# wangty537/raft_optical_flow

Hardware: AMD Instinct MI355X
Metric: image-pairs/s at Sintel 436x1024, 32 iters; corr-lookup GB/s vs HBM peak (higher is better)
Workload: dtype fp32 (convs: f16x3 split MFMA, fp32 accumulate); 1 GPU; RAFT-full inference, 436x1024 padded to 440x1024, 1 pair(s)/GPU/step, iters=32, all-pairs corr, hipGraph; global_batch=1, parallelism=frame-pair sharding x1

## Files before the change

include/raft_hip.h:

```cpp
#ifndef RAFT_HIP_H_
#define RAFT_HIP_H_

#include <stddef.h>

#ifdef __cplusplus
extern "C" {
#endif

#define RAFT_HIP_ABI_VERSION 19

#define RAFT_E_INVALID (-1)
#define RAFT_E_ALIGN (-2)

typedef void* raft_stream_t;

int raft_hip_abi_version(void);
const char* raft_hip_arch(void);
const char* raft_hip_last_error(void);
const char* raft_hip_source_hash(void);
int raft_debug_launch_span(int enable);
int raft_debug_launch_span_read(unsigned long long* host, int n);
int raft_debug_fill_lds_nan(raft_stream_t stream);

size_t raft_corr_pyramid_floats(int B, int H, int W, int num_levels);
// ... 128 lines not shown
int raft_conv2d_in_norm_ok(const raft_conv2d_params* p);
int raft_instnorm_merge(const float* part, int slots_per_image, int B, int C, int stats_ld, float eps,
                        float* stats, raft_stream_t stream);
size_t raft_instnorm_merge_ws_floats(int slots_per_image, int B, int C);
int raft_instnorm_merge_ws(const float* part, int slots_per_image, int B, int C, int stats_ld, float eps, void* ws,
                           float* stats, raft_stream_t stream);
size_t raft_instnorm_merge_counters(int B, int C);
int raft_instnorm_merge_fused(const float* part, int slots_per_image, int B, int C, int stats_ld, float eps, void* ws,
                              int* counters, float* stats, raft_stream_t stream);

int raft_conv2d_packed_shape(int mode, int n, int kh, int kw, int cin, int* n_pad, int* k_pad);
int raft_conv2d(const raft_conv2d_params* p, raft_stream_t stream);
int raft_conv2d_pair(const raft_conv2d_params* p0, const raft_conv2d_params* p1, raft_stream_t stream);
int raft_conv2d_set_halo_loaders(int nl);
int raft_conv2d_set_halo_ks(int ks);
int raft_conv2d_split_weight(const float* w, void* out, int n_pad, int k_pad, raft_stream_t stream);
size_t raft_conv2d_split_scaled_bytes(int n_pad, int k_pad);
int raft_conv2d_split_weight_scaled(const float* w, void* out, int n_pad, int k_pad, raft_stream_t stream);
int raft_conv2d_split_weight_prec(const float* w, void* out, int n_pad, int k_pad, int precision,
                                  raft_stream_t stream);

size_t raft_instnorm_workspace_floats(int B, int HW, int C);
int raft_instnorm_stats(const float* x, int ld, int B, int HW, int C, float eps, float* stats,
                        float* workspace, raft_stream_t stream);
int raft_groupnorm_stats(const float* x, int ld, int B, int HW, int C, int G, float eps, float* stats,
                         raft_stream_t stream);
int raft_norm_apply_affine(const float* x, int ld, const float* stats, const float* gamma, const float* beta,
                           const float* resid, int resid_ld, const float* resid_stats, const float* resid_gamma,
                           const float* resid_beta, int relu_mode, float* out, int out_ld, int B, int HW, int C,
                           raft_stream_t stream);
// ... 59 lines not shown
```

raft_optical_flow_amd/_lib.py:

```python
from __future__ import annotations

import ctypes
import os
import threading

_HERE = os.path.dirname(os.path.abspath(__file__))
LIB_PATH = os.environ.get("RAFT_HIP_LIB") or os.path.join(_HERE, "libraft_hip.so")

c_int = ctypes.c_int
c_float = ctypes.c_float
c_size_t = ctypes.c_size_t
c_long = ctypes.c_long
c_void_p = ctypes.c_void_p
c_char_p = ctypes.c_char_p
P = c_void_p

RAFT_CONV_VEC = 0
RAFT_CONV_GATHER = 1

PREC_FP32 = 0
PREC_F16X3 = 1
PREC_F16 = 2
PREC_BF16 = 3
PRECISIONS = {"fp32": PREC_FP32, "f16x3": PREC_F16X3, "f16": PREC_F16, "bf16": PREC_BF16}
# ... 125 lines not shown
    "raft_conv2d_stats_slots": (c_int, [ctypes.POINTER(ConvParams)]),
    "raft_conv2d_halo_tile_rows": (c_int, [ctypes.POINTER(ConvParams)]),
    "raft_conv2d_halo_tiles_per_wg": (c_int, [ctypes.POINTER(ConvParams)]),
    "raft_conv2d_form": (c_int, [ctypes.POINTER(ConvParams), ctypes.POINTER(ConvForm)]),
    "raft_conv2d_pair_form": (c_int, [ctypes.POINTER(ConvParams), ctypes.POINTER(ConvParams),
                                      ctypes.POINTER(ConvForm), ctypes.POINTER(c_int)]),
    "raft_debug_launch_span": (c_int, [c_int]),
    "raft_debug_launch_span_read": (c_int, [P, c_int]),
    "raft_conv2d_in_norm_ok": (c_int, [ctypes.POINTER(ConvParams)]),
    "raft_instnorm_merge": (c_int, [P, c_int, c_int, c_int, c_int, c_float, P, P]),
    "raft_instnorm_merge_ws_floats": (c_size_t, [c_int, c_int, c_int]),
    "raft_instnorm_merge_ws": (c_int, [P, c_int, c_int, c_int, c_int, c_float, P, P, P]),
    "raft_instnorm_merge_counters": (c_size_t, [c_int, c_int]),
    "raft_conv2d_set_halo_loaders": (c_int, [c_int]),
    "raft_conv2d_set_halo_ks": (c_int, [c_int]),
    "raft_instnorm_merge_fused": (c_int, [P, c_int, c_int, c_int, c_int, c_float, P, P, P, P]),
    "raft_conv2d_split_weight": (c_int, [P, P, c_int, c_int, P]),
    "raft_conv2d_split_weight_prec": (c_int, [P, P, c_int, c_int, c_int, P]),
    "raft_conv2d_split_scaled_bytes": (c_size_t, [c_int, c_int]),
    "raft_conv2d_split_weight_scaled": (c_int, [P, P, c_int, c_int, P]),
    "raft_instnorm_workspace_floats": (c_size_t, [c_int, c_int, c_int]),
    "raft_instnorm_stats": (c_int, [P, c_int, c_int, c_int, c_int, c_float, P, P, P]),
    "raft_groupnorm_stats": (c_int, [P, c_int, c_int, c_int, c_int, c_int, c_float, P, P]),
    "raft_norm_apply_affine": (c_int, [P, c_int, P, P, P, P, c_int, P, P, P, c_int, P, c_int, c_int, c_int, c_int, P]),
    "raft_instnorm_apply": (c_int, [P, c_int, P, P, c_int, P, c_int, P, c_int, c_int, c_int, c_int, P]),
    "raft_prep_images": (c_int, [P, P, P, c_int, c_int, c_int, P]),
    "raft_init_coords": (c_int, [P, P, c_int, c_int, c_int, P]),
    "raft_flow_from_coords": (c_int, [P, P, c_int, c_int, c_int, P]),
    "raft_convex_upsample": (c_int, [P, P, c_int, P, c_int, c_int, c_int, P]),
    "raft_upflow8": (c_int, [P, P, c_int, c_int, c_int, P]),
# ... 87 lines not shown
```

raft_optical_flow_amd/csrc/conv_common.hpp:

```cpp
#pragma once

#include "common.hpp"

namespace raft {
namespace {

using h4 = __attribute__((ext_vector_type(4))) _Float16;
using v4u = __attribute__((ext_vector_type(4))) unsigned;
using h8 = __attribute__((ext_vector_type(8))) _Float16;
using bf4 = __attribute__((ext_vector_type(4))) __bf16;
using bf8 = __attribute__((ext_vector_type(8))) __bf16;

__device__ __forceinline__ h4 to_bf16x4(const f32x4 x) {
  return __builtin_bit_cast(h4, __builtin_convertvector(x, bf4));
}

constexpr float SPLIT_SCALE = 2048.f;

__device__ __forceinline__ void split4(const f32x4 x, h4& hi, h4& lo) {
#pragma unroll
  for (int e = 0; e < 4; ++e) {
    const _Float16 h = (_Float16)x[e];
    hi[e] = h;
    lo[e] = (_Float16)((x[e] - (float)h) * SPLIT_SCALE);
// ... 134 lines not shown
  for (int j = 0; j < 4; ++j) {
    float x[4] = {v[4 * j], v[4 * j + 1], v[4 * j + 2], v[4 * j + 3]};
    quad_transpose(x);
    const int row = q == 0 ? rows[4 * j] : q == 1 ? rows[4 * j + 1] : q == 2 ? rows[4 * j + 2] : rows[4 * j + 3];
    const unsigned off = row >= 0 ? ((unsigned)row * (unsigned)ld + c0) * 4u : OFF_INVALID;
    __builtin_amdgcn_raw_buffer_store_b128(__builtin_bit_cast(v4u, f32x4{x[0], x[1], x[2], x[3]}), rs,
                                           full ? off : OFF_INVALID, 0, CPOL);
    if (part) {
#pragma unroll
      for (int i = 0; i < 4; ++i)
        if (nq + i < ncols) __builtin_amdgcn_raw_buffer_store_b32(__builtin_bit_cast(unsigned, x[i]), rs, off + 4u * i, 0, CPOL);
    }
  }
}

template <bool WT = false, int R0 = 0, int RN = 16>
__device__ __forceinline__ void tile_epilogue(const raft_conv2d_params& p, const int (&rows)[16], int n,
                                              const f32x16& acc) {
  static_assert(!WT || (R0 == 0 && RN == 16), "write-through epilogues store whole 16-row tiles");
  const bool ncol = n < p.n;
  const int nc = ncol ? n : p.n - 1;
  float v[16];
  const float bias = p.bias ? p.bias[nc] : 0.f;
#pragma unroll
  for (int r = R0; r < R0 + RN; ++r) v[r] = acc[r] + bias;
  if (p.add0) {
    float t[16];
    load_rows<WT, R0, RN>(p.add0, p.add0_ld, rows, nc, t);
#pragma unroll
    for (int r = R0; r < R0 + RN; ++r) v[r] += t[r];
  }
  float* dst = p.out;
  int ld = p.out_ld, col = n;
  const int epi = p.epilogue;
  if (epi == RAFT_EPI_LINEAR) {
#pragma unroll
    for (int r = R0; r < R0 + RN; ++r) v[r] *= p.alpha;
  } else if (epi == RAFT_EPI_RELU) {
#pragma unroll
    for (int r = R0; r < R0 + RN; ++r) v[r] = fmaxf(v[r], 0.f);
  } else if (epi == RAFT_EPI_RESID_RELU) {
    float t[16];
    load_rows<WT, R0, RN>(p.aux0, p.aux0_ld, rows, nc, t);
#pragma unroll
    for (int r = R0; r < R0 + RN; ++r) v[r] = fmaxf(t[r] + fmaxf(v[r], 0.f), 0.f);
  } else if (epi == RAFT_EPI_GRU_ZR) {
    if (nc < p.split) {
#pragma unroll
      for (int r = R0; r < R0 + RN; ++r) v[r] = sigmoid_bf(v[r]);
    } else {
      col = nc - p.split;
      float t[16];
      load_rows<WT, R0, RN>(p.aux0, p.aux0_ld, rows, col, t);
#pragma unroll
      for (int r = R0; r < R0 + RN; ++r) v[r] = sigmoid_bf(v[r]) * t[r];
      dst = p.out1;
      ld = p.out1_ld;
    }
  } else if (epi == RAFT_EPI_GRU_Q) {
    float h[16], z[16];
    load_rows<WT, R0, RN>(p.aux0, p.aux0_ld, rows, nc, h);
    load_rows<WT, R0, RN>(p.aux1, p.aux1_ld, rows, nc, z);
#pragma unroll
    for (int r = R0; r < R0 + RN; ++r) v[r] = (1.0f - z[r]) * h[r] + z[r] * tanh_bf(v[r]);
  } else if (epi == RAFT_EPI_TANH_RELU) {
    if (nc < p.split) {
#pragma unroll
      for (int r = R0; r < R0 + RN; ++r) v[r] = tanh_bf(v[r]);
    } else {
#pragma unroll
      for (int r = R0; r < R0 + RN; ++r) v[r] = fmaxf(v[r], 0.f);
      dst = p.out1;
      ld = p.out1_ld;
      col = n - p.split;
    }
  } else if (epi == RAFT_EPI_ADD_TO_OUT) {
    float t[16];
// ... 7 lines not shown
    for (int r = R0; r < R0 + RN; ++r) big |= ncol && rows[r] >= 0 && fabsf(v[r]) > RAFT_RANGE_LIMIT;
    if (big) *p.range_flag = 1;
  }
  if (WT && (((uintptr_t)dst) & 15) == 0 && (ld & 3) == 0) {
    store_tile16<WT ? CPOL_SC1 : 0>(dst, ld, (long)p.batch * p.out_h * p.out_w, rows, col, n - (threadIdx.x & 3), p.n, v);
    return;
  }
#pragma unroll
  for (int r = R0; r < R0 + RN; ++r)
    if (ncol && rows[r] >= 0) {
      if constexpr (WT)
        __hip_atomic_store(dst + eidx(rows[r], ld, col), v[r], __ATOMIC_RELAXED, __HIP_MEMORY_SCOPE_AGENT);
      else
        dst[eidx(rows[r], ld, col)] = v[r];
    }
}

__device__ __forceinline__ f32x4 tile_stats_vals(const int (&rows)[16], const f32x16& acc, float bias) {
  float s = 0.f, c = 0.f;
#pragma unroll
  for (int r = 0; r < 16; ++r) {
    s += rows[r] >= 0 ? acc[r] + bias : 0.f;
    c += rows[r] >= 0 ? 1.f : 0.f;
  }
  s += __shfl_xor(s, 32);
  c += __shfl_xor(c, 32);
  const float mean = c > 0.f ? s / c : 0.f;
  float m2 = 0.f;
#pragma unroll
  for (int r = 0; r < 16; ++r) {
// ... 66 lines not shown

struct HaloOperands {
  raft_conv2d_params p;
  int k_pad, n_pad;
  unsigned w_bytes, in0_bytes, in1_bytes;
};

using ConvForm = struct raft_conv2d_form;

int conv_halo_launch(const HaloOperands& o, hipStream_t s, ConvForm* form = nullptr);
int conv_halo_launch_pair(const HaloOperands& o0, const HaloOperands& o1, hipStream_t s, ConvForm* form = nullptr);
int conv_stem_launch(const raft_conv2d_params& p, int k_pad, hipStream_t s, ConvForm* form = nullptr);
int conv_halo_stats_slots(const HaloOperands& o);
bool conv_halo_covers(const HaloOperands& o);
int conv_halo_tile_rows(const HaloOperands& o);
int conv_halo_tiles_per_wg(const HaloOperands& o);
bool conv_halo_norm_ok(const HaloOperands& o);
int conv_stem_stats_slots(const raft_conv2d_params& p, int k_pad);

}
```

raft_optical_flow_amd/csrc/conv_gemm.hip:

```cpp
#include "conv_common.hpp"

namespace raft {
namespace {

constexpr int BM = 64;
constexpr int BN = 64;
constexpr int BK = 32;
constexpr int LDSK = BK + 4;
constexpr int STAGE = (BM + BN) * LDSK;
constexpr int MAX_GATHER_K = 1024;
#ifndef CONV_SCHED
#define CONV_SCHED 1
#endif
#ifndef GEMM_NS
#define GEMM_NS 2
#endif

struct ConvArgs {
  raft_conv2d_params p;
  int M;
  int K;
  int ctot;
  int cpad;
  int taps;
// ... 898 lines not shown
extern "C" int raft_conv2d_in_norm_ok(const raft_conv2d_params* pp) {
  ConvArgs a;
  HaloOperands o;
  if (!pp || conv_prepare(pp, a, o)) return 0;
  return pp->mode == RAFT_CONV_VEC && pp->n > 4 && conv_halo_norm_ok(o) ? 1 : 0;
}

extern "C" int raft_conv2d_halo_tile_rows(const raft_conv2d_params* pp) {
  ConvArgs a;
  HaloOperands o;
  if (!pp || conv_prepare(pp, a, o)) return 0;
  if (pp->mode != RAFT_CONV_VEC || small_n(*pp)) return 0;
  return conv_halo_tile_rows(o);
}

extern "C" int raft_conv2d_halo_tiles_per_wg(const raft_conv2d_params* pp) {
  ConvArgs a;
  HaloOperands o;
  if (!pp || conv_prepare(pp, a, o)) return 0;
  if (pp->mode != RAFT_CONV_VEC || small_n(*pp)) return 0;
  return conv_halo_tiles_per_wg(o);
}

extern "C" int raft_conv2d_stats_slots(const raft_conv2d_params* pp) {
  ConvArgs a;
  HaloOperands o;
  if (!pp || conv_prepare(pp, a, o)) return 0;
  const raft_conv2d_params& p = *pp;
  if (p.epilogue != RAFT_EPI_LINEAR || p.alpha != 1.0f || p.add0 || (p.n <= 4 && p.mode == RAFT_CONV_VEC)) return 0;
  if (p.mode == RAFT_CONV_VEC) {
// ... 52 lines not shown
```

raft_optical_flow_amd/csrc/conv_halo.hip:

```cpp
#include <atomic>
#include <type_traits>

#include "conv_common.hpp"

namespace raft {
namespace {

constexpr int HTW = 16;
constexpr int HTH = 8;
constexpr int HTH_BIG = 16;
constexpr int HALO_LDS = 160 * 1024;

struct HaloArgs {
  raft_conv2d_params p;
  const float* inv_scale;
  int K;
  int nch;
  int nk;
  int gn;
  int tx_n, ty_n;
  unsigned w_bytes, in0_bytes, in1_bytes;
};

struct HaloLaunch {
  HaloArgs a[2];
  int sp0, sp1;
  int m;
  int grid0;
};

constexpr int patch_slots(int T, int U, int D, int late = 0) {
  for (int pa = 1; pa < 16; ++pa) {
    bool ok = true;
    for (int c = pa; c < 512 && ok; ++c) {
      const int last = (c - pa) * T + T - 1;
      const int rd = last == 0 ? -1 : (last - 1) / U;
// ... 20 lines not shown
                                                                              : 2;
#else
  static constexpr int D = halo_lds_bytes(T, U, 3, BNT, PI, WR) <= LB ? 3 : 2;
#endif
  static constexpr int PA = patch_slots(T, U, D);
#ifndef HALO_WX
#define HALO_WX 0
#endif
  static constexpr int DW = (T > 1 && D == 3 && HALO_WX > 0 &&
                             U * (D + HALO_WX + 1) * BNT * WR + PA * PI * 1024 + 16 * 1024 <= LB)
                                ? D + HALO_WX
                                : D;
  static constexpr int SB = U * (DW + 1);
  static constexpr int LDS_B = SB * BNT * WR, LDS_A = PA * PI * 1024;
};

#ifdef STAMPS
__device__ unsigned long long g_hstamp[8 * 16384];
__device__ unsigned long long g_lstamp[8 * 16384];
__device__ __forceinline__ unsigned long long hstamp_real() {
  unsigned long long t;
  __builtin_amdgcn_sched_barrier(0);
  asm volatile("s_memrealtime %0\n\ts_waitcnt lgkmcnt(0)" : "=s"(t)::"memory");
  __builtin_amdgcn_sched_barrier(0);
  return t;
}
__device__ __forceinline__ unsigned long long hstamp_now() {
  unsigned long long t;
  __builtin_amdgcn_sched_barrier(0);
  asm volatile("s_memtime %0\n\ts_waitcnt lgkmcnt(0)" : "=s"(t)::"memory");
// ... 50 lines not shown
  constexpr int SGB = (ENC && NL == 8) ? 0 : HALO_SGB;
#ifndef HALO_RELAX
#define HALO_RELAX 1
#endif
  constexpr int NRD1 = NSUB * 2 * (X3 ? 2 : 1) + MF * 2 * (X3 ? 2 : 1);
  constexpr bool RELAX = HALO_RELAX && SGB > 0 && LSPLIT && !MT && patch_slots(T, U, D, 1) == PA && NRD1 <= 15;
  static_assert(D >= 2 && C::LDS_B + C::LDS_A <= C::LB, "LDS budget");
  static_assert(KS == 1 || (KS == 2 && !MT && !ENC && LSPLIT && SGB > 0 && MF == 1 && NSUB <= 2 && (NL == 4 || NL == 8) &&
                            SB % 2 == 0 && 8 * 4096 <= C::LDS_B + C::LDS_A && (DW == D || !KSW) && NBI % NWPC == 0 &&
                            NWPC >= 1),
                "the K-split form: one tile of 32 x 64 blocks on the pre-split path, 4 loaders");
  static_assert(NWP >= 1 && NBI % NWP == 0, "a wave's weight pieces lie in one K-step");
  static_assert(U % 2 == 0 && (T == 1 || T >= U), "fragment parity; at most one chunk start per load set");
  constexpr int NORM_BYTES = halo_norm_bytes<KH, KW, BNT, PREC, ENC>(C::LDS_B, C::LDS_A, D);
  static_assert(NORM_BYTES == 0 || NORM_BYTES >= 256 * 8, "room for one image's norm table");

#ifdef STAMPS
  const unsigned long long r_entry = hstamp_real(), c_entry = hstamp_now();
#endif
  const int lane = threadIdx.x & 63;
  const int w = __builtin_amdgcn_readfirstlane(threadIdx.x >> 6);
  constexpr int NCW = 4 * KS;
  const bool loader = w >= NCW;
  const int lw = loader ? w - NCW : w;
  const int wc = w & 3;
  const int kp = KS > 1 ? (w >> 2) & (KS - 1) : 0;

  const HaloArgs& a = args[prob];
  const raft_conv2d_params& p = a.p;
  const int per = a.tx_n * a.ty_n;
// ... 272 lines not shown
              nnew += pcw;
            }
            if constexpr (DW == D) {
              issue_weights(s + D);
              nnew += NWP;
            }
          }
          wait_vm_n(s + 1 < NS ? nnew : 0);
          __builtin_amdgcn_s_barrier();
        }
        wait_vm<0>();
        if constexpr (KS > 1) __builtin_amdgcn_s_barrier();
        return;
      }
#endif
      constexpr int PMAX = (U * D + T - 1) / T + 1;
      Staged pv[PMAX];
      int pks[PMAX], pcs[PMAX];
      int nst = 0;
#pragma unroll
      for (int u = 0; u < D; ++u) {
        int kt, c;
        if (set_chunk(u, kt, c)) {
#pragma unroll
          for (int k = 0; k < PMAX; ++k)
            if (k == nst) {
              load_patch(kt, c, pv[k]);
              pks[k] = kt;
              pcs[k] = c;
            }
// ... 2 lines not shown
      }
      wait_vm<0>();
#pragma unroll
      for (int k = 0; k < PMAX; ++k)
        if (k < nst) store_patch(pks[k], pcs[k], pv[k]);
      __builtin_amdgcn_s_waitcnt(0xC07F);
      __builtin_amdgcn_s_barrier();
      int pend_k = -1, pend_c = 0;
#ifdef STAMPS
      unsigned long long l_st = 0, l_ld = 0, l_w = 0, l_wait = 0, l_bar = 0, l0 = hstamp_now(), l1;
      const unsigned long long l_loop = l0;
#define LSTAMP(acc) (l1 = hstamp_now(), acc += l1 - l0, l0 = l1)
#else
#define LSTAMP(acc)
#endif
      for (int s = 0; s < NS; ++s) {
        if (pend_k >= 0) {
          wait_vm<LNWP>();
          store_patch(pend_k, pend_c, pv[0]);
          pend_k = -1;
        }
        LSTAMP(l_st);
        int nnew = 0;
        if (s + D < NS) {
          int kt, c;
          if (set_chunk(s + D, kt, c)) {
            load_patch(kt, c, pv[0]);
            pend_k = kt;
            pend_c = c;
            nnew = 2 * TI;
          }
// ... 6 lines not shown
          }
        }
        if constexpr (DW > D && !KSW) {
          if (s + DW < NS) {
            issue_weights(s + DW);
            nnew += NWP;
          }
        }
        LSTAMP(l_w);
        wait_vm_n(s + 1 < NS ? nnew + (DW - D) * NWP : 0);
        __builtin_amdgcn_s_waitcnt(0xC07F);
        LSTAMP(l_wait);
        __builtin_amdgcn_s_barrier();
        LSTAMP(l_bar);
      }
#undef LSTAMP
#ifdef STAMPS
      {
        const unsigned lid = blockIdx.x * NL + lw;
        if (lane == 0 && lid < 16384) {
          unsigned long long* g = g_lstamp + lid * 8;
          g[0] = l_st;
          g[1] = l_ld;
          g[2] = l_w;
          g[3] = l_wait;
          g[4] = l_bar;
          g[5] = hstamp_now() - l_loop;
          g[6] = 1;
        }
      }
// ... 44 lines not shown
    for (int f = 0; f < MF; ++f)
#pragma unroll
      for (int sb = 0; sb < NSUB; ++sb) acc[f][sb] = f32x16{};
#pragma unroll
    for (int f = 0; f < AXF; ++f)
#pragma unroll
      for (int sb = 0; sb < AXS; ++sb) accx[f][sb] = f32x16{};
  };
  clear_acc();
  int b_bs = kp;
  int a_t = 0, a_ky = 0, a_kx = 0, a_ps = 0;
  struct Frag {
    h8 ah[MF][2], al[MF][2];
    h8 bh[NSUB][2], bl[NSUB][2];
  };
  f32x4 av[MF][4];
  auto read_b = [&](Frag& F) {
    const char* Bb = smem + b_bs * (BNT * WROW);
#pragma unroll
    for (int sb = 0; sb < NSUB; ++sb) {
#pragma unroll
      for (int qq = 0; qq < 2; ++qq) {
        F.bh[sb][qq] = *reinterpret_cast<const h8*>(Bb + (cb + sb * 32 + m) * WROW + (((2 * h + qq) ^ bsw) << 4));
        if constexpr (X3)
          F.bl[sb][qq] = *reinterpret_cast<const h8*>(Bb + (cb + sb * 32 + m) * WROW + (((4 + 2 * h + qq) ^ bsw) << 4));
      }
    }
    b_bs = b_bs + KS >= SB ? b_bs + KS - SB : b_bs + KS;
  };
  auto advance_a = [&]() {
// ... 121 lines not shown
#pragma unroll
          for (int r = 0; r < 16; ++r) acc[f][sb][r] += accx[f][sb][r] * (1.0f / SPLIT_SCALE);
    }
    f32x4 stv[NSUB];
    const int oh = __builtin_amdgcn_readfirstlane(p.out_h), ow = __builtin_amdgcn_readfirstlane(p.out_w);
    const int rowb = t.b * oh;
#pragma unroll
    for (int f = 0; f < MF; ++f) {
      int rows[16];
#pragma unroll
      for (int r = 0; r < 16; ++r) {
        const int mm = (r & 3) + 8 * (r >> 2) + 4 * h;
        const int y = t.y0 + 2 * (wm * MF + f) + (mm >> 4), x = t.x0 + (mm & 15);
        rows[r] = ((y < oh) & (x < ow)) ? (rowb + y) * ow + x : -1;
      }
#pragma unroll
      for (int sb = 0; sb < NSUB; ++sb) tile_epilogue<false>(p, rows, t.n0 + cb + sb * 32 + m, acc[f][sb]);
      if constexpr (ENC) {
        if (p.stats_part) {
#pragma unroll
          for (int sb = 0; sb < NSUB; ++sb) {
            const int n = t.n0 + sb * 32 + m;
            const f32x4 v = tile_stats_vals(rows, acc[f][sb], p.bias ? p.bias[n < p.n ? n : 0] : 0.f);
            stv[sb] = f == 0 ? v : stats_combine(stv[sb], v);
            if (f == MF - 1) stats_write(p, n, (long)t.st * 4 + w, stv[sb]);
          }
        }
      }
    }
  };

  auto epilogue_ks2 = [&](const Tile& t) {
// ... 39 lines not shown
      else
        tile_epilogue<false, 0, 8>(p, rows, t.n0 + cb + m, keep);
    } else if constexpr (KS > 1) {
      if constexpr (X3 && !SC) {
#pragma unroll
        for (int sb = 0; sb < NSUB; ++sb)
#pragma unroll
          for (int r = 0; r < 16; ++r) acc[0][sb][r] += accx[0][sb][r] * (1.0f / SPLIT_SCALE);
      }
      f32x16 keep, send;
#pragma unroll
      for (int r = 0; r < 16; ++r) {
        keep[r] = kp ? acc[0][1][r] : acc[0][0][r];
        send[r] = kp ? acc[0][0][r] : acc[0][1][r];
      }
      f32x4* mine = reinterpret_cast<f32x4*>(smem + (wc * 2 + kp) * 4096) + lane * 4;
      const f32x4* theirs = reinterpret_cast<const f32x4*>(smem + (wc * 2 + (kp ^ 1)) * 4096) + lane * 4;
#pragma unroll
      for (int q = 0; q < 4; ++q)
        mine[q ^ (lane & 3)] = f32x4{send[4 * q], send[4 * q + 1], send[4 * q + 2], send[4 * q + 3]};
      __builtin_amdgcn_s_waitcnt(0xC07F);
      __builtin_amdgcn_s_barrier();
#pragma unroll
      for (int q = 0; q < 4; ++q) {
        const f32x4 o = theirs[q ^ (lane & 3)];
#pragma unroll
        for (int i = 0; i < 4; ++i) keep[4 * q + i] += o[i];
      }
      const int oh = __builtin_amdgcn_readfirstlane(p.out_h), ow = __builtin_amdgcn_readfirstlane(p.out_w);
      const int rowb = t.b * oh;
      int rows[16];
#pragma unroll
      for (int r = 0; r < 16; ++r) {
        const int mm = (r & 3) + 8 * (r >> 2) + 4 * h;
        const int y = t.y0 + 2 * wm + (mm >> 4), x = t.x0 + (mm & 15);
        rows[r] = ((y < oh) & (x < ow)) ? (rowb + y) * ow + x : -1;
      }
      tile_epilogue<false>(p, rows, t.n0 + cb + kp * 32 + m, keep);
    }
  };

  if constexpr (KS > 1) {
    if (kp) advance_a();
  }
  const WPiecesC wpc = wpieces_c(KSW ? w : 0);
  if constexpr (KSW) {
#pragma unroll
    for (int u = 0; u < DW; ++u) issue_weights_c(u, wpc);
    wait_vm<NWPC * (DW - 2)>();
  } else if constexpr (KS > 1) {
    if (NL == 8 || kp == 0) {
#pragma unroll
      for (int u = 0; u < DW; ++u) issue_weights(u);
// ... 189 lines not shown
      g[1] = r_exit;
      g[2] = c_loop - c_entry;
      g[3] = t_cmp;
      g[4] = t_wait + t_bar;
      g[5] = t_epi;
      g[6] = c_exit - c_entry;
    }
  }
#endif
}

template <int KH, int KW, int BNT, int PREC, bool ENC = false, int TH = HTH, bool MT = false, int NL = 4, int KS = 1>
__global__ __launch_bounds__(64 * (4 * KS + NL)) void conv_halo_kernel(HaloLaunch hl) {
  using C = HaloCfg<KH, KW, BNT, PREC == RAFT_PREC_F16X3 ? 128 : 64, TH>;
  constexpr int NORM_BYTES = halo_norm_bytes<KH, KW, BNT, PREC, ENC>(C::LDS_B, C::LDS_A, C::D);
  __shared__ __attribute__((aligned(1024))) char smem[C::LDS_B + C::LDS_A + NORM_BYTES];
  int g = xcd_tile(blockIdx.x, gridDim.x);
  const int prob = g >= hl.grid0 ? 1 : 0;
  g -= prob * hl.grid0;
  const int gn = hl.a[prob].gn;
  if constexpr (MT) {
    const int st0 = (g / gn) * hl.m;
    const int ntl = min(hl.m, (prob ? hl.sp1 : hl.sp0) - st0);
    halo_body<KH, KW, BNT, PREC, ENC, TH, true, NL>(hl.a, prob, g % gn, st0, ntl, smem);
  } else {
    halo_body<KH, KW, BNT, PREC, ENC, TH, false, NL, KS>(hl.a, prob, g % gn, g / gn, 1, smem);
  }
}

std::atomic<int> g_halo_nl{0};
bool halo_nl8() {
// ... 9 lines not shown
#define HALO_KS2_NL8 0
#endif
#ifndef HALO_KS2_BN32
#define HALO_KS2_BN32 0
#endif
std::atomic<int> g_halo_ks{0};
bool halo_ks2() {
  int v = g_halo_ks.load(std::memory_order_relaxed);
  if (v == 0) {
    const char* e = getenv("RAFT_HALO_KS2");
    v = e && e[0] == '0' ? 1 : 2;
    g_halo_ks.store(v, std::memory_order_relaxed);
  }
  return v == 2;
}
bool halo_nl8_enc() {
  const char* e = getenv("RAFT_HALO_NL8_ENC");
  return !(e && e[0] == '0');
}
constexpr bool halo_no_mt(int prec, int taps, int bn) { return prec != RAFT_PREC_F16X3 && taps == 9 && bn == 128; }

template <int KH, int KW, int BNT, int PREC, bool ENC, int TH, bool MT, int NL = 4, int KS = 1>
void halo_start(const HaloLaunch& l, dim3 grid, hipStream_t s, ConvForm* q) {
  if (q) {
    *q = ConvForm{};
    q->kernel = RAFT_CONV_KERNEL_HALO;
    q->tile_rows = TH;
    q->tile_cols = BNT;
    q->tiles_per_wg = MT ? l.m : 1;
    q->loader_waves = NL;
// ... 109 lines not shown
  const int kh = p.kh, kw = p.kw;
  const bool shape = (kh == 1 && kw == 1) || (kh == 3 && kw == 3) || (kh == 1 && kw == 5) || (kh == 5 && kw == 1);
  if (!shape || p.pad_h != (kh - 1) / 2 || p.pad_w != (kw - 1) / 2) return false;
  if (p.out_h != p.in_h || p.out_w != p.in_w || p.n <= 4) return false;
  a.p = p;
  a.inv_scale = nullptr;
  a.K = o.k_pad;
  a.nch = o.k_pad / (kh * kw) / 32;
  a.nk = a.nch * kh * kw;
  a.tx_n = cdiv(p.out_w, HTW);
  a.ty_n = cdiv(p.out_h, HTH);
  a.w_bytes = o.w_bytes;
  a.in0_bytes = o.in0_bytes;
  a.in1_bytes = o.in1_bytes;
  a.gn = 0;
  return true;
}

long halo_spatial(const HaloArgs& a) { return (long)a.p.batch * a.tx_n * a.ty_n; }

long halo_big_min() {
  static const long v = [] {
    const char* e = getenv("RAFT_HALO_BIG_MIN");
    return e ? atol(e) : 1L;
  }();
  return v;
}
double halo_big_cost() {
  static const double v = [] {
    const char* e = getenv("RAFT_HALO_BIG_COST");
// ... 163 lines not shown
}
#endif

extern "C" int raft_conv2d_set_halo_loaders(int nl) {
  const int prev = halo_nl8() ? 8 : 4;
  if (nl == 4 || nl == 8) g_halo_nl.store(nl, std::memory_order_relaxed);
  return prev;
}

extern "C" int raft_conv2d_set_halo_ks(int ks) {
  const int prev = halo_ks2() ? 2 : 1;
  if (ks == 1 || ks == 2) g_halo_ks.store(ks, std::memory_order_relaxed);
  return prev;
}

bool conv_halo_norm_ok(const HaloOperands& o) {
  HaloArgs a;
  if (!halo_enabled() || !halo_problem(o, a)) return false;
  const raft_conv2d_params& p = o.p;
  return p.kh == 3 && p.kw == 3 && p.in0_c <= 256 && HaloCfg<3, 3, 64>::D == 3 && HaloCfg<3, 3, 32>::D == 3;
}

long halo_wide_min() {
  static const long v = [] {
    const char* e = getenv("RAFT_HALO_WIDE_MIN");
    return e ? atol(e) : 256L;
  }();
  return v;
}
bool halo_wide_enabled() {
// ... 21 lines not shown
  bool wide;
  return halo_pick(o, a, wide);
}

bool conv_halo_covers(const HaloOperands& o) {
  HaloArgs a;
  return halo_enabled() && halo_problem(o, a);
}

int conv_halo_stats_slots(const HaloOperands& o) {
  HaloArgs a;
  if (!halo_enabled() || !halo_problem(o, a)) return 0;
  if (!((o.p.kh == 1 && o.p.kw == 1) || (o.p.kh == 3 && o.p.kw == 3))) return 0;
  const int th = halo_pick_th(o, false);
  return a.tx_n * cdiv(o.p.out_h, th) * 4;
}

static bool halo_plan(const HaloOperands& o, HaloLaunch& l, int& bn, int& th, long& wgs) {
  if (!halo_enabled() || !halo_problem(o, l.a[0])) return false;
  const long spatial = halo_spatial(l.a[0]);
  bool wide;
  th = halo_pick(o, l.a[0], wide);
  bn = th == HTH_BIG ? 64 : wide ? 128 : spatial * (o.n_pad / 64) > 128 ? 64 : 32;
  halo_set_th(o, l.a[0], th);
  l.a[0].gn = o.n_pad / bn;
  const long tiles = halo_spatial(l.a[0]) * l.a[0].gn;
  if (tiles >= (1L << 31)) return false;
  l.a[1] = l.a[0];
  wgs = halo_plan_grid(l, bn, th, false);
  return true;
}

int conv_halo_tiles_per_wg(const HaloOperands& o) {
  HaloLaunch l;
  int bn, th;
  long wgs;
  return halo_plan(o, l, bn, th, wgs) ? l.m : 0;
}

int conv_halo_launch(const HaloOperands& o, hipStream_t s, ConvForm* q) {
  HaloLaunch l;
  int bn, th;
  long wgs;
  if (!halo_plan(o, l, bn, th, wgs)) return 1;
  launch_halo(l, bn, th, wgs, s, q);
  return 0;
}

int conv_halo_launch_pair(const HaloOperands& o0, const HaloOperands& o1, hipStream_t s, ConvForm* q) {
  HaloLaunch l;
  if (!halo_enabled() || !halo_problem(o0, l.a[0]) || !halo_problem(o1, l.a[1])) return 1;
  const raft_conv2d_params &p0 = o0.p, &p1 = o1.p;
  if (p0.kh != p1.kh || p0.kw != p1.kw || p0.precision != p1.precision) return 1;
  const int th = halo_pick_th(o0, false);
  if (halo_pick_th(o1, false) != th) return 1;
  halo_set_th(o0, l.a[0], th);
  halo_set_th(o1, l.a[1], th);
  const long s0 = halo_spatial(l.a[0]), s1 = halo_spatial(l.a[1]);
  const int bn = th == HTH_BIG ? 64 : s0 * (o0.n_pad / 64) + s1 * (o1.n_pad / 64) > 128 ? 64 : 32;
  if (o0.n_pad % bn || o1.n_pad % bn) return 1;
  l.a[0].gn = o0.n_pad / bn;
  l.a[1].gn = o1.n_pad / bn;
  const long t0 = s0 * l.a[0].gn, tiles = t0 + s1 * l.a[1].gn;
  if (tiles >= (1L << 31)) return 1;
  launch_halo(l, bn, th, halo_plan_grid(l, bn, th, true), s, q);
  if (q) q[1] = q[0];
  return 0;
}


}
```

Baseline: 148.8 image-pairs/s.

## Stage GRU epilogue operands into LDS via DMA during halo conv K-loop tail

For f16x3 1x5/5x1 halo convolutions with GRU_Q/GRU_ZR epilogues, the last three K-loop steps are peeled off. The add0/aux0/aux1 epilogue operand tiles are then DMA'd into LDS slots (ring and patch buffers) that are freed as the loop drains. The epilogue reads these operands from LDS instead of issuing scattered global loads after the MMA loop, which hides that latency behind the final K-steps. The cost is extra barriers, more LDS for the K-split variant, and intricate slot-reuse invariants, guarded by static_asserts and an env toggle that defaults on.

```diff
diff --git a/include/raft_hip.h b/include/raft_hip.h
--- a/include/raft_hip.h
+++ b/include/raft_hip.h
@@ -166,6 +166,8 @@
 int raft_conv2d_pair(const raft_conv2d_params* p0, const raft_conv2d_params* p1, raft_stream_t stream);
 int raft_conv2d_set_halo_loaders(int nl);
 int raft_conv2d_set_halo_ks(int ks);
+int raft_conv2d_set_halo_epi_stage(int on);
+int raft_conv2d_epi_staged(const raft_conv2d_params* p);
 int raft_conv2d_split_weight(const float* w, void* out, int n_pad, int k_pad, raft_stream_t stream);
 size_t raft_conv2d_split_scaled_bytes(int n_pad, int k_pad);
 int raft_conv2d_split_weight_scaled(const float* w, void* out, int n_pad, int k_pad, raft_stream_t stream);
diff --git a/raft_optical_flow_amd/_lib.py b/raft_optical_flow_amd/_lib.py
--- a/raft_optical_flow_amd/_lib.py
+++ b/raft_optical_flow_amd/_lib.py
@@ -163,6 +163,8 @@
     "raft_instnorm_merge_counters": (c_size_t, [c_int, c_int]),
     "raft_conv2d_set_halo_loaders": (c_int, [c_int]),
     "raft_conv2d_set_halo_ks": (c_int, [c_int]),
+    "raft_conv2d_set_halo_epi_stage": (c_int, [c_int]),
+    "raft_conv2d_epi_staged": (c_int, [ctypes.POINTER(ConvParams)]),
     "raft_instnorm_merge_fused": (c_int, [P, c_int, c_int, c_int, c_int, c_float, P, P, P, P]),
     "raft_conv2d_split_weight": (c_int, [P, P, c_int, c_int, P]),
     "raft_conv2d_split_weight_prec": (c_int, [P, P, c_int, c_int, c_int, P]),
diff --git a/raft_optical_flow_amd/csrc/conv_common.hpp b/raft_optical_flow_amd/csrc/conv_common.hpp
--- a/raft_optical_flow_amd/csrc/conv_common.hpp
+++ b/raft_optical_flow_amd/csrc/conv_common.hpp
@@ -172,10 +172,29 @@
   }
 }
 
-template <bool WT = false, int R0 = 0, int RN = 16>
-__device__ __forceinline__ void tile_epilogue(const raft_conv2d_params& p, const int (&rows)[16], int n,
-                                              const f32x16& acc) {
+struct EpiLds {
+  const char* base;
+  int add0, aux0, aux1;
+};
+template <int R0, int RN>
+__device__ __forceinline__ void lds_rows(const char* base, int off, float (&t)[16]) {
+#pragma unroll
+  for (int r = R0; r < R0 + RN; ++r) t[r] = *reinterpret_cast<const float*>(base + off + 128 * ((r & 3) + 8 * (r >> 2)));
+}
+template <bool WT, int R0, int RN, bool STG>
+__device__ __forceinline__ void epi_rows(const float* g, int ld, const int (&rows)[16], int col, const char* lbase,
+                                         int off, float (&t)[16]) {
+  if constexpr (STG)
+    lds_rows<R0, RN>(lbase, off, t);
+  else
+    load_rows<WT, R0, RN>(g, ld, rows, col, t);
+}
+
+template <bool WT, int R0, int RN, bool STG>
+__device__ __forceinline__ void tile_epilogue_t(const raft_conv2d_params& p, const int (&rows)[16], int n,
+                                                const f32x16& acc, const EpiLds& lds) {
   static_assert(!WT || (R0 == 0 && RN == 16), "write-through epilogues store whole 16-row tiles");
+  static_assert(!(WT && STG), "staged operands are plain loads' values");
   const bool ncol = n < p.n;
   const int nc = ncol ? n : p.n - 1;
   float v[16];
@@ -184,7 +203,7 @@
   for (int r = R0; r < R0 + RN; ++r) v[r] = acc[r] + bias;
   if (p.add0) {
     float t[16];
-    load_rows<WT, R0, RN>(p.add0, p.add0_ld, rows, nc, t);
+    epi_rows<WT, R0, RN, STG>(p.add0, p.add0_ld, rows, nc, lds.base, lds.add0, t);
 #pragma unroll
     for (int r = R0; r < R0 + RN; ++r) v[r] += t[r];
   }
@@ -209,7 +228,7 @@
     } else {
       col = nc - p.split;
       float t[16];
-      load_rows<WT, R0, RN>(p.aux0, p.aux0_ld, rows, col, t);
+      epi_rows<WT, R0, RN, STG>(p.aux0, p.aux0_ld, rows, col, lds.base, lds.aux0, t);
 #pragma unroll
       for (int r = R0; r < R0 + RN; ++r) v[r] = sigmoid_bf(v[r]) * t[r];
       dst = p.out1;
@@ -217,8 +236,8 @@
     }
   } else if (epi == RAFT_EPI_GRU_Q) {
     float h[16], z[16];
-    load_rows<WT, R0, RN>(p.aux0, p.aux0_ld, rows, nc, h);
-    load_rows<WT, R0, RN>(p.aux1, p.aux1_ld, rows, nc, z);
+    epi_rows<WT, R0, RN, STG>(p.aux0, p.aux0_ld, rows, nc, lds.base, lds.aux0, h);
+    epi_rows<WT, R0, RN, STG>(p.aux1, p.aux1_ld, rows, nc, lds.base, lds.aux1, z);
 #pragma unroll
     for (int r = R0; r < R0 + RN; ++r) v[r] = (1.0f - z[r]) * h[r] + z[r] * tanh_bf(v[r]);
   } else if (epi == RAFT_EPI_TANH_RELU) {
@@ -256,6 +275,11 @@
       else
         dst[eidx(rows[r], ld, col)] = v[r];
     }
+}
+template <bool WT = false, int R0 = 0, int RN = 16>
+__device__ __forceinline__ void tile_epilogue(const raft_conv2d_params& p, const int (&rows)[16], int n,
+                                              const f32x16& acc) {
+  tile_epilogue_t<WT, R0, RN, false>(p, rows, n, acc, EpiLds{nullptr, -1, -1, -1});
 }
 
 __device__ __forceinline__ f32x4 tile_stats_vals(const int (&rows)[16], const f32x16& acc, float bias) {
@@ -352,6 +376,7 @@
 int conv_halo_stats_slots(const HaloOperands& o);
 bool conv_halo_covers(const HaloOperands& o);
 int conv_halo_tile_rows(const HaloOperands& o);
+int conv_halo_epi_staged(const HaloOperands& o);
 int conv_halo_tiles_per_wg(const HaloOperands& o);
 bool conv_halo_norm_ok(const HaloOperands& o);
 int conv_stem_stats_slots(const raft_conv2d_params& p, int k_pad);
diff --git a/raft_optical_flow_amd/csrc/conv_gemm.hip b/raft_optical_flow_amd/csrc/conv_gemm.hip
--- a/raft_optical_flow_amd/csrc/conv_gemm.hip
+++ b/raft_optical_flow_amd/csrc/conv_gemm.hip
@@ -936,6 +936,14 @@
   return conv_halo_tile_rows(o);
 }
 
+extern "C" int raft_conv2d_epi_staged(const raft_conv2d_params* pp) {
+  ConvArgs a;
+  HaloOperands o;
+  if (!pp || conv_prepare(pp, a, o)) return 0;
+  if (pp->mode != RAFT_CONV_VEC || small_n(*pp)) return 0;
+  return conv_halo_epi_staged(o);
+}
+
 extern "C" int raft_conv2d_halo_tiles_per_wg(const raft_conv2d_params* pp) {
   ConvArgs a;
   HaloOperands o;
diff --git a/raft_optical_flow_amd/csrc/conv_halo.hip b/raft_optical_flow_amd/csrc/conv_halo.hip
--- a/raft_optical_flow_amd/csrc/conv_halo.hip
+++ b/raft_optical_flow_amd/csrc/conv_halo.hip
@@ -20,6 +20,7 @@
   int gn;
   int tx_n, ty_n;
   unsigned w_bytes, in0_bytes, in1_bytes;
+  int stage;
 };
 
 struct HaloLaunch {
@@ -70,6 +71,46 @@
   static constexpr int SB = U * (DW + 1);
   static constexpr int LDS_B = SB * BNT * WR, LDS_A = PA * PI * 1024;
 };
+
+constexpr int STAGE_TILE = 128 * 32 * 4;
+constexpr int stage_ring_sets(int D, int DW) { return D == 3 && DW == D ? 2 : 0; }
+constexpr int stage_chunk(int NS, int T, int U) { return (NS * U + T - 1) / T; }
+constexpr bool stage_patch_free(int T, int U, int D, int PA, int late, int lead) {
+  for (int NS = D; NS < 1024; ++NS) {
+    const int prev = stage_chunk(NS, T, U) - PA;
+    if (prev < 0) continue;
+    const int last = prev * T + T - 1;
+    const int rd = last == 0 ? -1 : (last - 1) / U;
+    if (rd + late > NS - lead - 1) return false;
+  }
+  return true;
+}
+#ifndef HALO_STG_KS1
+#define HALO_STG_KS1 1
+#endif
+#ifndef HALO_STG_KS2
+#define HALO_STG_KS2 1
+#endif
+constexpr bool halo_stg_form(int prec, int taps, int th, bool mt, int bnt, int nl, int ks) {
+  return prec == RAFT_PREC_F16X3 && taps == 5 && th == HTH && !mt &&
+         ((HALO_STG_KS1 && ks == 1 && bnt == 32 && nl == 8) || (HALO_STG_KS2 && ks == 2 && bnt == 64 && nl == 4));
+}
+#ifndef HALO_NOLSPLIT
+#define HALO_NOLSPLIT 0
+#endif
+#ifndef HALO_KSW
+#define HALO_KSW 0
+#endif
+constexpr bool HALO_STG_BUILD = !HALO_NOLSPLIT && !HALO_KSW && !HALO_WX;
+template <int KH, int KW, int BNT, int PREC, bool ENC, int TH, bool MT, int NL, int KS>
+constexpr bool halo_stg() {
+  using C = HaloCfg<KH, KW, BNT, PREC == RAFT_PREC_F16X3 ? 128 : 64, TH>;
+  return HALO_STG_BUILD && !ENC && halo_stg_form(PREC, KH * KW, TH, MT, BNT, NL, KS) && C::D == 3 && C::DW == C::D;
+}
+template <int KH, int KW, int BNT, int PREC, bool ENC, int TH, bool MT, int NL, int KS>
+constexpr int halo_stage_extra() {
+  return halo_stg<KH, KW, BNT, PREC, ENC, TH, MT, NL, KS>() && KS == 2 ? STAGE_TILE : 0;
+}
 
 #ifdef STAMPS
 __device__ unsigned long long g_hstamp[8 * 16384];
@@ -150,6 +191,19 @@
   static_assert(U % 2 == 0 && (T == 1 || T >= U), "fragment parity; at most one chunk start per load set");
   constexpr int NORM_BYTES = halo_norm_bytes<KH, KW, BNT, PREC, ENC>(C::LDS_B, C::LDS_A, D);
   static_assert(NORM_BYTES == 0 || NORM_BYTES >= 256 * 8, "room for one image's norm table");
+  constexpr bool STG = halo_stg<KH, KW, BNT, PREC, ENC, TH, MT, NL, KS>();
+  constexpr int SLOT = U * BNT * WROW;
+  constexpr int STG_X = C::LDS_B + C::LDS_A;
+  static_assert(!STG || (LSPLIT && !KSW && DW == D && NORM_BYTES == 0 && MF == 1 && NSUB == KS && WN == 1),
+                "staging: the pre-split one-tile loop, loaders issuing the weights");
+  static_assert(!STG || (stage_ring_sets(D, DW) == 2 && SLOT >= STAGE_TILE && SLOT % 4096 == 0),
+                "staging: two phantom load sets certified by the K loop's last barrier, a tile each");
+  constexpr int PSTEP = stage_patch_free(T, U, D, PA, RELAX ? 1 : 0, D) ? 0 : 1;
+  static_assert(!STG || (PI * 1024 >= STAGE_TILE && stage_patch_free(T, U, D, PA, RELAX ? 1 : 0, D - PSTEP)),
+                "staging: the patch slot of the first chunk past the loop is retired when its tile is issued");
+  static_assert(!STG || KS == 1 || (4 * KS * 4096 <= 2 * SLOT && D + 1 >= 4 && STG_X + STAGE_TILE <= C::LB),
+                "staging (K-split): the exchange fits the slots of sets NS + 2, NS + 3; a tile behind the rings");
+  static_assert((STAGE_TILE / 1024) % NL == 0, "a staged tile's 1-KiB pieces split evenly over the loaders");
 
 #ifdef STAMPS
   const unsigned long long r_entry = hstamp_real(), c_entry = hstamp_now();
@@ -452,6 +506,47 @@
         return;
       }
 #endif
+      const int stg = STG ? __builtin_amdgcn_readfirstlane(a.stage) : 0;
+      auto stage_tile = [&](const float* g, int ld, int ncols, int col0, int dst) -> int {
+        const int oh = p.out_h, ow = p.out_w;
+        const unsigned bytes = ((unsigned)(p.batch * oh * ow - 1) * (unsigned)ld + (unsigned)ncols) * 4u;
+        const __amdgpu_buffer_rsrc_t rs = make_rsrc(g, bytes);
+        constexpr int NP = STAGE_TILE / 1024 / NL;
+#ifdef HALO_ABL_STG_NODMA
+        return 0;
+#endif
+#pragma unroll
+        for (int k = 0; k < NP; ++k) {
+          const int i = lw + NL * k, tp = 8 * i + (lane >> 3);
+          const int y = tile0.y0 + (tp >> 4), x = tile0.x0 + (tp & 15);
+          const int row = ((y < oh) & (x < ow)) ? (tile0.b * oh + y) * ow + x : 0;
+          dma16(rs, smem + dst + i * 1024, ((unsigned)row * (unsigned)ld + (unsigned)(col0 + 4 * (lane & 7))) * 4u, 0);
+        }
+        return NP;
+      };
+      auto stage_issue = [&](int step) -> int {
+        int n = 0;
+        if constexpr (STG) {
+          const int ring = ((NS + step) % (D + 1)) * SLOT;
+          const int patch = C::LDS_B + (stage_chunk(NS, T, U) % PA) * (PI * 1024);
+          if constexpr (KS == 1) {
+            if (stg & (step == 0 ? 2 : 4))
+              n += stage_tile(step == 0 ? p.aux0 : p.aux1, step == 0 ? p.aux0_ld : p.aux1_ld, p.n, tile0.n0, ring);
+            if (step == PSTEP && (stg & 1)) n += stage_tile(p.add0, p.add0_ld, p.n, tile0.n0, patch);
+          } else {
+            if (stg & 1) n += stage_tile(p.add0, p.add0_ld, p.n, tile0.n0 + 32 * step, ring);
+            if (stg & 2) {
+#pragma unroll
+              for (int k = 0; k < 2; ++k) {
+                const int c0 = tile0.n0 + 32 * k - p.split;
+                if (step == (k ? 0 : PSTEP) && c0 >= 0)
+                  n += stage_tile(p.aux0, p.aux0_ld, p.n - p.split, c0, k ? STG_X : patch);
+              }
+            }
+          }
+        }
+        return n;
+      };
       constexpr int PMAX = (U * D + T - 1) / T + 1;
       Staged pv[PMAX];
       int pks[PMAX], pcs[PMAX];
@@ -484,7 +579,8 @@
 #else
 #define LSTAMP(acc)
 #endif
-      for (int s = 0; s < NS; ++s) {
+      const int ns_main = (STG && stg) ? NS - 3 : NS;
+      for (int s = 0; s < ns_main; ++s) {
         if (pend_k >= 0) {
           wait_vm<LNWP>();
           store_patch(pend_k, pend_c, pv[0]);
@@ -521,6 +617,22 @@
         __builtin_amdgcn_s_barrier();
         LSTAMP(l_bar);
       }
+      if constexpr (STG) {
+        if (stg) {
+          if (pend_k >= 0) {
+            wait_vm<LNWP>();
+            store_patch(pend_k, pend_c, pv[0]);
+          }
+          const int n0 = stage_issue(0);
+          wait_vm_n(n0);
+          __builtin_amdgcn_s_waitcnt(0xC07F);
+          __builtin_amdgcn_s_barrier();
+          wait_vm_n(n0 + stage_issue(1));
+          __builtin_amdgcn_s_barrier();
+          wait_vm<0>();
+          __builtin_amdgcn_s_barrier();
+        }
+      }
 #undef LSTAMP
 #ifdef STAMPS
       {
@@ -595,6 +707,7 @@
     h8 ah[MF][2], al[MF][2];
     h8 bh[NSUB][2], bl[NSUB][2];
   };
+  static_assert(NRD1 * (int)sizeof(h8) * (X3 ? 1 : 2) == (int)sizeof(Frag), "NRD1 = the fragment reads of a K-step");
   f32x4 av[MF][4];
   auto read_b = [&](Frag& F) {
     const char* Bb = smem + b_bs * (BNT * WROW);
@@ -746,8 +859,19 @@
         const int y = t.y0 + 2 * (wm * MF + f) + (mm >> 4), x = t.x0 + (mm & 15);
         rows[r] = ((y < oh) & (x < ow)) ? (rowb + y) * ow + x : -1;
       }
-#pragma unroll
-      for (int sb = 0; sb < NSUB; ++sb) tile_epilogue<false>(p, rows, t.n0 + cb + sb * 32 + m, acc[f][sb]);
+      if constexpr (STG && KS == 1) {
+        if (__builtin_amdgcn_readfirstlane(a.stage)) {
+          const int lo = (32 * wm + 4 * h) * 128 + 4 * m;
+          const int ring0 = (NS % (D + 1)) * SLOT, ring1 = ((NS + 1) % (D + 1)) * SLOT;
+          const int patch = C::LDS_B + (stage_chunk(NS, T, U) % PA) * (PI * 1024);
+          tile_epilogue_t<false, 0, 16, true>(p, rows, t.n0 + m, acc[0][0], EpiLds{smem, patch + lo, ring0 + lo, ring1 + lo});
+        } else {
+          tile_epilogue<false>(p, rows, t.n0 + m, acc[0][0]);
+        }
+      } else {
+#pragma unroll
+        for (int sb = 0; sb < NSUB; ++sb) tile_epilogue<false>(p, rows, t.n0 + cb + sb * 32 + m, acc[f][sb]);
+      }
       if constexpr (ENC) {
         if (p.stats_part) {
 #pragma unroll
@@ -817,8 +941,12 @@
         keep[r] = kp ? acc[0][1][r] : acc[0][0][r];
         send[r] = kp ? acc[0][0][r] : acc[0][1][r];
       }
-      f32x4* mine = reinterpret_cast<f32x4*>(smem + (wc * 2 + kp) * 4096) + lane * 4;
-      const f32x4* theirs = reinterpret_cast<const f32x4*>(smem + (wc * 2 + (kp ^ 1)) * 4096) + lane * 4;
+      auto xslot = [&](int e) {
+        if constexpr (STG) return ((NS + 2 + e / (SLOT / 4096)) % (D + 1)) * SLOT + (e % (SLOT / 4096)) * 4096;
+        return e * 4096;
+      };
+      f32x4* mine = reinterpret_cast<f32x4*>(smem + xslot(wc * 2 + kp)) + lane * 4;
+      const f32x4* theirs = reinterpret_cast<const f32x4*>(smem + xslot(wc * 2 + (kp ^ 1))) + lane * 4;
 #pragma unroll
       for (int q = 0; q < 4; ++q)
         mine[q ^ (lane & 3)] = f32x4{send[4 * q], send[4 * q + 1], send[4 * q + 2], send[4 * q + 3]};
@@ -839,7 +967,18 @@
         const int y = t.y0 + 2 * wm + (mm >> 4), x = t.x0 + (mm & 15);
         rows[r] = ((y < oh) & (x < ow)) ? (rowb + y) * ow + x : -1;
       }
-      tile_epilogue<false>(p, rows, t.n0 + cb + kp * 32 + m, keep);
+      if constexpr (STG) {
+        if (__builtin_amdgcn_readfirstlane(a.stage)) {
+          const int lo = (32 * wm + 4 * h) * 128 + 4 * m;
+          const int ring = ((NS + kp) % (D + 1)) * SLOT;
+          const int patch = C::LDS_B + (stage_chunk(NS, T, U) % PA) * (PI * 1024);
+          tile_epilogue_t<false, 0, 16, true>(p, rows, t.n0 + kp * 32 + m, keep, EpiLds{smem, ring + lo, (kp ? STG_X : patch) + lo, 0});
+        } else {
+          tile_epilogue<false>(p, rows, t.n0 + kp * 32 + m, keep);
+        }
+      } else {
+        tile_epilogue<false>(p, rows, t.n0 + cb + kp * 32 + m, keep);
+      }
     }
   };
 
@@ -1059,7 +1198,8 @@
 __global__ __launch_bounds__(64 * (4 * KS + NL)) void conv_halo_kernel(HaloLaunch hl) {
   using C = HaloCfg<KH, KW, BNT, PREC == RAFT_PREC_F16X3 ? 128 : 64, TH>;
   constexpr int NORM_BYTES = halo_norm_bytes<KH, KW, BNT, PREC, ENC>(C::LDS_B, C::LDS_A, C::D);
-  __shared__ __attribute__((aligned(1024))) char smem[C::LDS_B + C::LDS_A + NORM_BYTES];
+  constexpr int STAGE_X = halo_stage_extra<KH, KW, BNT, PREC, ENC, TH, MT, NL, KS>();
+  __shared__ __attribute__((aligned(1024))) char smem[C::LDS_B + C::LDS_A + NORM_BYTES + STAGE_X];
   int g = xcd_tile(blockIdx.x, gridDim.x);
   const int prob = g >= hl.grid0 ? 1 : 0;
   g -= prob * hl.grid0;
@@ -1099,6 +1239,49 @@
   }
   return v == 2;
 }
+#ifndef HALO_EPI_STAGE_DEFAULT
+#define HALO_EPI_STAGE_DEFAULT 1
+#endif
+std::atomic<int> g_halo_epi_stage{0};
+bool halo_epi_stage() {
+  int v = g_halo_epi_stage.load(std::memory_order_relaxed);
+  if (v == 0) {
+    const char* e = getenv("RAFT_HALO_EPI_STAGE");
+    v = e && (e[0] == '0' || e[0] == '1') ? (e[0] == '1' ? 2 : 1) : (HALO_EPI_STAGE_DEFAULT ? 2 : 1);
+    g_halo_epi_stage.store(v, std::memory_order_relaxed);
+  }
+  return v == 2;
+}
+static_assert(HaloCfg<1, 5, 32>::D == 3 && HaloCfg<5, 1, 32>::D == 3 && HaloCfg<1, 5, 64>::D == 3 &&
+                  HaloCfg<5, 1, 64>::D == 3,
+              "halo_stage_mask's loop-length floor");
+int halo_stage_mask(const HaloArgs& a, const ConvForm& f) {
+  const raft_conv2d_params& p = a.p;
+  if (!HALO_STG_BUILD || !halo_epi_stage()) return 0;
+  if (f.kernel != RAFT_CONV_KERNEL_HALO || p.stats_part || p.in_norm) return 0;
+  if (!halo_stg_form(p.precision, p.kh * p.kw, f.tile_rows, f.tiles_per_wg > 1, f.tile_cols, f.loader_waves,
+                     f.compute_waves_per_simd))
+    return 0;
+  const int U = f.tile_cols == 32 ? 4 : 2;
+  if (halo_nkp(a.nk, U, 5, false) / U < 3 || p.n % f.tile_cols) return 0;
+  auto dma_ok = [](const float* g, int ld) { return g && ((uintptr_t)g & 15) == 0 && ld % 4 == 0; };
+  int m = 0;
+  if (f.compute_waves_per_simd == 1 && p.epilogue == RAFT_EPI_GRU_Q) {
+    if (!dma_ok(p.aux0, p.aux0_ld) || !dma_ok(p.aux1, p.aux1_ld)) return 0;
+    m = 6;
+  } else if (f.compute_waves_per_simd == 2 && p.epilogue == RAFT_EPI_GRU_ZR) {
+    if (!dma_ok(p.aux0, p.aux0_ld)) return 0;
+    m = 2;
+  } else {
+    return 0;
+  }
+  if (p.add0) {
+    if (!dma_ok(p.add0, p.add0_ld)) return 0;
+    m |= 1;
+  }
+  return m;
+}
+
 bool halo_nl8_enc() {
   const char* e = getenv("RAFT_HALO_NL8_ENC");
   return !(e && e[0] == '0');
@@ -1238,6 +1421,7 @@
   a.in0_bytes = o.in0_bytes;
   a.in1_bytes = o.in1_bytes;
   a.gn = 0;
+  a.stage = 0;
   return true;
 }
 
@@ -1431,6 +1615,12 @@
   return prev;
 }
 
+extern "C" int raft_conv2d_set_halo_epi_stage(int on) {
+  const int prev = halo_epi_stage() ? 1 : 0;
+  if (on == 0 || on == 1) g_halo_epi_stage.store(on ? 2 : 1, std::memory_order_relaxed);
+  return prev;
+}
+
 bool conv_halo_norm_ok(const HaloOperands& o) {
   HaloArgs a;
   if (!halo_enabled() || !halo_problem(o, a)) return false;
@@ -1482,6 +1672,13 @@
   if (!((o.p.kh == 1 && o.p.kw == 1) || (o.p.kh == 3 && o.p.kw == 3))) return 0;
   const int th = halo_pick_th(o, false);
   return a.tx_n * cdiv(o.p.out_h, th) * 4;
+}
+
+static void halo_set_stage(HaloLaunch& l, int bn, int th, long wgs, bool pair) {
+  ConvForm f;
+  launch_halo(l, bn, th, wgs, nullptr, &f);
+  l.a[0].stage = halo_stage_mask(l.a[0], f);
+  l.a[1].stage = pair ? halo_stage_mask(l.a[1], f) : l.a[0].stage;
 }
 
 static bool halo_plan(const HaloOperands& o, HaloLaunch& l, int& bn, int& th, long& wgs) {
@@ -1511,8 +1708,18 @@
   int bn, th;
   long wgs;
   if (!halo_plan(o, l, bn, th, wgs)) return 1;
+  halo_set_stage(l, bn, th, wgs, false);
   launch_halo(l, bn, th, wgs, s, q);
   return 0;
+}
+
+int conv_halo_epi_staged(const HaloOperands& o) {
+  HaloLaunch l;
+  int bn, th;
+  long wgs;
+  if (!halo_plan(o, l, bn, th, wgs)) return 0;
+  halo_set_stage(l, bn, th, wgs, false);
+  return l.a[0].stage;
 }
 
 int conv_halo_launch_pair(const HaloOperands& o0, const HaloOperands& o1, hipStream_t s, ConvForm* q) {
@@ -1531,7 +1738,9 @@
   l.a[1].gn = o1.n_pad / bn;
   const long t0 = s0 * l.a[0].gn, tiles = t0 + s1 * l.a[1].gn;
   if (tiles >= (1L << 31)) return 1;
-  launch_halo(l, bn, th, halo_plan_grid(l, bn, th, true), s, q);
+  const long wgs = halo_plan_grid(l, bn, th, true);
+  halo_set_stage(l, bn, th, wgs, true);
+  launch_halo(l, bn, th, wgs, s, q);
   if (q) q[1] = q[0];
   return 0;
 }
```

Measured after the change: 149.6 image-pairs/s (median of 6 runs). Within noise of the previous version (+0.5%).
